# gnosisguild/stylus-zkvm-verifiers

Measured on AMD Instinct MI355X. Metric: Groth16 proofs verified/sec (BN254), higher is better.
Workload: dtype u32

## Files before the change

### stylus_zkvm_verifiers_amd/csrc/k_gt.hip

```cpp
#include "zkv_internal.h"

namespace zkv {

__global__ __launch_bounds__(64) void k_gt_bases(const VkRaw* __restrict__ raw, const VkTables* __restrict__ t, uint32_t* __restrict__ tab, uint32_t* __restrict__ mconst,
                                                 uint32_t* __restrict__ scratch, uint32_t nw0, uint32_t nw1) {
    if (threadIdx.x != 0) return;
    const uint32_t b = blockIdx.x;
    uint32_t* sc = scratch + (size_t)b * 12 * 96;
    MRef fm = m_ref(sc, 1), tm = m_ref(sc + 96, 1), E = m_ref(sc + 2 * 96, 1), Y1 = m_ref(sc + 3 * 96, 1), Y3 = m_ref(sc + 4 * 96, 1), Y4 = m_ref(sc + 5 * 96, 1),
         W = m_ref(sc + 6 * 96, 1), acc = m_ref(sc + 9 * 96, 1);
    Fp2 gx, gy;
    gx.c0 = fp_from_raw(raw->gamma[0]); gx.c1 = fp_from_raw(raw->gamma[1]);
    gy.c0 = fp_from_raw(raw->gamma[2]); gy.c1 = fp_from_raw(raw->gamma[3]);
    G1Norm n;
    n.lxs = n.lys = n.cxs = n.cys = fp_zero();
    if (b == 2) {
        MRef out = m_ref(mconst, 1), ab = m_ref(const_cast<uint32_t*>(t->f_alpha_beta), 1);
        if (t->base_inf) { f12m_copy(out, ab); return; }
        const Fp iy = fp_inv(t->base.y);
        n.axs = fp_mul(t->base.x, iy); n.ays = iy;
        miller_loop_m((const VkTables*)nullptr, 0, n, gx, gy, fm, tm);
        f12m_mul(out, fm, ab);
        return;
    }
    const uint32_t nw = b ? nw1 : nw0, row0 = b ? nw0 : 0u;
    const uint32_t ici = raw->var_ic[b];
    const Fp px = fp_from_raw(raw->ic[ici][0]), py = fp_from_raw(raw->ic[ici][1]);
    const Fp iy = fp_inv(py);
    n.axs = fp_mul(px, iy); n.ays = iy;
    miller_loop_m((const VkTables*)nullptr, 0, n, gx, gy, fm, tm);
    (void)final_exp_is_one_m(fm, E, Y1, Y3, Y4, W, acc);
#pragma unroll 1
    for (uint32_t j = 0; j < nw; j++) {
        f12m_copy(m_ref(tab + gt_row_word(row0 + j), 1), acc);
#pragma unroll 1
        for (uint32_t k = 0; k < GT_WINDOW_BITS; k++) f12m_cyclo_sqr(acc);
    }
}

__global__ __launch_bounds__(64) void k_gt_level(uint32_t* __restrict__ tab, uint32_t rows, uint32_t level) {
    const uint32_t cnt = level == GT_WINDOW_BITS - 1 ? 1u : 1u << level;
    const uint32_t tt = blockIdx.x * 64 + threadIdx.x, row = blockIdx.y;
    if (tt >= cnt || row >= rows) return;
    const uint32_t d = (1u << level) + tt;
    uint32_t* base = tab + gt_row_word(row);
    MRef dst = m_ref(base + (size_t)(d - 1) * GT_ENTRY_WORDS, 1), src = m_ref(base + (size_t)((d >> 1) - 1) * GT_ENTRY_WORDS, 1), one = m_ref(base, 1);
    f12m_copy(dst, src);
    f12m_cyclo_sqr(dst);
    if (d & 1u) f12m_mul(dst, dst, one);
}

void launch_gt_bases(const VkRaw* d_raw, const VkTables* d_tab, uint32_t* tab, uint32_t* mconst, uint32_t* scratch, uint32_t nw0, uint32_t nw1, hipStream_t s) {
    hipLaunchKernelGGL(k_gt_bases, dim3(3), dim3(64), 0, s, d_raw, d_tab, tab, mconst, scratch, nw0, nw1);
}
void launch_gt_level(uint32_t* tab, uint32_t rows, uint32_t level, hipStream_t s) {
    if (!rows || level < 1 || level >= GT_WINDOW_BITS) return;
    const uint32_t cnt = level == GT_WINDOW_BITS - 1 ? 1u : 1u << level;
    hipLaunchKernelGGL(k_gt_level, dim3((cnt + 63) / 64, rows), dim3(64), 0, s, tab, rows, level);
}

}
```

### stylus_zkvm_verifiers_amd/csrc/zkv_capi.hip

```cpp
#include <hip/hip_runtime.h>
#include <condition_variable>
#include <functional>
#include <memory>
#include <mutex>
#include <new>
#include <math.h>
#include <stdio.h>
#include <stdlib.h>
#include <string.h>
#include <system_error>
#include <thread>
#include <utility>
#include <vector>

#include "../../include/zkv.h"
#include "../../include/zkv_groth16_set.h"
#include "../../include/zkv_sp1_gateway.h"
#include "../../include/zkv_sp1_gateway_wire.h"
#include "../../include/zkv_sp1_gateway_keys.h"
#include "../../include/zkv_plonk_keys.h"
#include "../../include/zkv_plonk_set.h"
#include "../../include/zkv_plonk_set_agg.h"
#include "../../include/zkv_diag_primitive.h"
#include "../../include/zkv_diag_prep.h"
// ... 429 lines not shown
        hipMalloc(&c->ws.f, sizeof(uint32_t) * WS_F_WORDS * cap) != hipSuccess ||
        hipMalloc(&c->ws.fe, sizeof(uint32_t) * WS_FE_WORDS * cap) != hipSuccess ||
        hipMalloc(&c->ws.flags, sizeof(uint32_t) * cap) != hipSuccess || hipMalloc(&c->ws.g2bad, sizeof(uint32_t) * cap) != hipSuccess ||
        hipMalloc(&c->d_a, 32 * cap) != hipSuccess || hipMalloc(&c->d_b, 32 * cap) != hipSuccess ||
        hipMalloc(&c->d_status, cap) != hipSuccess || hipMalloc(&c->d_recv, 4 * cap) != hipSuccess ||
        hipMalloc(&c->d_off, sizeof(uint64_t) * (cap + 1)) != hipSuccess ||
        hipMalloc(&c->d_pvoff, sizeof(uint64_t) * (cap + 1)) != hipSuccess ||
        hipMalloc(&c->d_inst_idx, sizeof(uint32_t) * cap) != hipSuccess ||
        hipMalloc(&c->d_len, sizeof(uint32_t) * cap) != hipSuccess || hipMalloc(&c->d_pvlen, sizeof(uint32_t) * cap) != hipSuccess ||
        hipMalloc(&c->d_kind, cap) != hipSuccess || hipMalloc(&c->d_cdoff[0], sizeof(uint64_t) * (cap + 1)) != hipSuccess ||
        hipMalloc(&c->d_cdoff[1], sizeof(uint64_t) * (cap + 1)) != hipSuccess ||
        ((is_plonk(c) || c->vm == ZKV_VM_PLONK_SET) && hipMalloc(&c->d_plonk_tab, sizeof(uint32_t) * PLONK_TAB_WORDS * cap) != hipSuccess)) {
        (void)hipGetLastError();
        return ZKV_ERR_OOM;
    }
    c->ws.cap = cap;
    return agg_reserve(c);
}
static int gt_window_bits() {
    const char* e = getenv("ZKV_GT_WINDOW_BITS");
    if (!e || !strcmp(e, "20")) return (int)GT_WINDOW_BITS;
    return !strcmp(e, "0") ? 0 : -1;
}
static size_t gt_max_bytes() {
    const char* e = getenv("ZKV_GT_MAX_BYTES");
    return e ? (size_t)strtoull(e, nullptr, 10) : ~(size_t)0;
}
static int gt_maybe_build(zkv_ctx* c, size_t n) {
    if (c->gt_tried || (c->vm != ZKV_VM_SP1 && c->vm != ZKV_VM_RISC0) || c->vk_invalid || !c->d_tab) return ZKV_OK;
    const size_t per = n < chunk_capacity() ? n : chunk_capacity();
    if (!(c->lanes == 2 || (c->lanes == 0 && per > wide_below()))) return ZKV_OK;
    const int bits = gt_window_bits();
    if (bits < 0) return ZKV_ERR_INVALID_ARG;
    c->gt_tried = true;
    if (bits == 0) return ZKV_OK;
    VkRaw raw;
    if (c->vm == ZKV_VM_RISC0) host::fill_vk_risc0(raw, c->control_root_0, c->control_root_1, c->control_id);
    else host::fill_vk_sp1(raw);
    if (raw.n_var != GT_MAX_SIG || !raw.var_windows[0] || !raw.var_windows[1]) return ZKV_OK;
    const uint32_t nw0 = gt_windows(8 * raw.var_windows[0]), nw1 = gt_windows(8 * raw.var_windows[1]), rows = nw0 + nw1;
    if (nw0 > GT_MAX_WINDOWS || nw1 > GT_MAX_WINDOWS) return ZKV_OK;
    const size_t bytes = (size_t)rows * GT_ROW_BYTES;
    if (bytes > gt_max_bytes()) return ZKV_OK;
    VkRaw* d_raw = nullptr; uint32_t* d_scr = nullptr;
    hipEvent_t e0 = nullptr, e1 = nullptr;
    bool ok = hipMalloc(&c->d_gt, bytes) == hipSuccess && hipMalloc(&c->d_gt_const, sizeof(uint32_t) * GT_ENTRY_WORDS) == hipSuccess &&
              hipMalloc(&d_raw, sizeof(VkRaw)) == hipSuccess && hipMalloc(&d_scr, sizeof(uint32_t) * GT_SETUP_SCRATCH_WORDS) == hipSuccess &&
              hipEventCreate(&e0) == hipSuccess && hipEventCreate(&e1) == hipSuccess;
    if (ok) {
        ok = hipMemcpyAsync(d_raw, &raw, sizeof raw, hipMemcpyHostToDevice, c->stream) == hipSuccess;
        (void)hipEventRecord(e0, c->stream);
        launch_gt_bases(d_raw, c->d_tab, c->d_gt, c->d_gt_const, d_scr, nw0, nw1, c->stream);
        for (uint32_t level = 1; level < GT_WINDOW_BITS; level++) launch_gt_level(c->d_gt, rows, level, c->stream);
        (void)hipEventRecord(e1, c->stream);
        ok = ok && hipGetLastError() == hipSuccess && hipStreamSynchronize(c->stream) == hipSuccess;
        if (ok) (void)hipEventElapsedTime(&c->gt_build_ms, e0, e1);
    }
    (void)hipGetLastError();
    if (e0) (void)hipEventDestroy(e0);
    if (e1) (void)hipEventDestroy(e1);
    if (d_raw) (void)hipFree(d_raw);
    if (d_scr) (void)hipFree(d_scr);
    if (!ok) {
        if (c->d_gt) (void)hipFree(c->d_gt);
        if (c->d_gt_const) (void)hipFree(c->d_gt_const);
        c->d_gt = c->d_gt_const = nullptr;
        return ZKV_OK;
    }
    c->gt = GtTab{c->d_gt, c->d_gt_const, {nw0, nw1}};
    c->gt_bytes = bytes;
    return ZKV_OK;
}
static int ctx_ready(zkv_ctx* c, size_t n, bool verify = true) {
    int rc = ctx_device_init(c);
    if (rc == ZKV_OK) rc = ctx_reserve(c, n ? n : 1);
    if (rc == ZKV_OK && verify) rc = gt_maybe_build(c, n ? n : 1);
    return rc;
}
static int grow(uint8_t** p, size_t* cap, size_t need) {
    if (need <= *cap) return ZKV_OK;
    if (*p) (void)hipFree(*p);
    *p = nullptr; *cap = 0;
    size_t want = need + need / 4 + 4096;
    if (hipMalloc(p, want) != hipSuccess) { (void)hipGetLastError(); return ZKV_ERR_OOM; }
    *cap = want;
    return ZKV_OK;
}

static int order_after_previous(zkv_ctx* c, hipStream_t s) {
    if (c->has_done) HIP_TRY(hipStreamWaitEvent(s, c->ev_done, 0));
    c->agg_look = true;
    return ZKV_OK;
}
static int mark_done(zkv_ctx* c, hipStream_t s) {
    HIP_TRY(hipEventRecord(c->ev_done, s));
    c->has_done = true;
    return ZKV_OK;
}

static size_t agg_min() {
    const char* e = getenv("ZKV_AGG_MIN");
    size_t v = e ? (size_t)strtoull(e, nullptr, 10) : (size_t)131072;
    return v < 64 ? 64 : v;
}
static uint32_t agg_group(uint32_t sub) {
    const char* e = getenv("ZKV_AGG_GROUP");
// ... 2547 lines not shown
    return rc;
}

static_assert(ZKV_DIAG_PREP_SIGNALS == MAX_VAR, "zkv_diag_prep.h documents MAX_VAR signal rows");
ZKV_EXPORT int zkv_diag_prep_signals(zkv_ctx* c, size_t n, uint32_t* signals, uint32_t* flags) {
    if (!c || !signals || !flags || n == 0) return ZKV_ERR_INVALID_ARG;
    if (is_sharded(c) || (c->vm != ZKV_VM_RISC0 && c->vm != ZKV_VM_SP1) || c->agg_on) return ZKV_ERR_INVALID_ARG;
    int nd = 0;
    if (hipGetDeviceCount(&nd) != hipSuccess || nd <= 0) { (void)hipGetLastError(); return ZKV_ERR_NO_DEVICE; }
    if (c->device < 0 || c->device >= nd || !device_is_gfx950(c->device)) return ZKV_ERR_NO_DEVICE;
    std::lock_guard<std::mutex> lk(c->mu);
    if (!c->dev_ready || !c->ws.prep || n > c->last_chunk_n || n > c->ws.cap) return ZKV_ERR_INVALID_ARG;
    HIP_TRY(hipSetDevice(c->device));
    HIP_TRY(hipDeviceSynchronize());
    const size_t rows = (size_t)8 * MAX_VAR;
    std::vector<uint32_t> t(rows * n);
    HIP_TRY(hipMemcpy2D(t.data(), 4 * n, c->ws.prep + (size_t)64 * c->ws.cap, 4 * c->ws.cap, 4 * n, rows, hipMemcpyDeviceToHost));
    HIP_TRY(hipMemcpy(flags, c->ws.flags, 4 * n, hipMemcpyDeviceToHost));
    for (size_t j = 0; j < n; j++)
        for (size_t r = 0; r < rows; r++) signals[j * rows + r] = t[r * n + j];
    return ZKV_OK;
}

ZKV_EXPORT int zkv_ctx_vm(const zkv_ctx* c) { return c ? c->vm : ZKV_ERR_INVALID_ARG; }
ZKV_EXPORT int zkv_ctx_set_lanes_per_proof(zkv_ctx* c, int lanes) {
    if (!c || (lanes != 0 && lanes != 2 && lanes != 16 && lanes != 64 && lanes != 128)) return ZKV_ERR_INVALID_ARG;
    if (is_sharded(c)) { for (auto* k : c->shards) { const int rc = zkv_ctx_set_lanes_per_proof(k, lanes); if (rc != ZKV_OK) return rc; } return ZKV_OK; }
    if (c->vm == ZKV_VM_MIXED) {
        for (auto* k : c->kid) { const int rc = zkv_ctx_set_lanes_per_proof(k, lanes); if (rc != ZKV_OK) return rc; }
    }
    for (auto* k : c->gw_route) { if (!k) continue; const int rc = zkv_ctx_set_lanes_per_proof(k, lanes); if (rc != ZKV_OK) return rc; }
    if (c->gw_group) { const int rc = zkv_ctx_set_lanes_per_proof(c->gw_group, lanes); if (rc != ZKV_OK) return rc; }
    std::lock_guard<std::mutex> lk(c->mu);
    c->lanes = lanes;
    return ZKV_OK;
}
ZKV_EXPORT int zkv_diag_gt_info(zkv_ctx* c, uint64_t* out6) {
    if (!c || !out6) return ZKV_ERR_INVALID_ARG;
    std::lock_guard<std::mutex> lk(c->mu);
    out6[0] = c->gt.tab ? 1 : 0; out6[1] = c->gt.nw[0]; out6[2] = c->gt.nw[1]; out6[3] = c->gt_bytes;
    out6[4] = (uint64_t)(c->gt_build_ms * 1000.0f); out6[5] = c->gt_tried ? 1 : 0;
    return ZKV_OK;
}
ZKV_EXPORT int zkv_diag_gt_read(zkv_ctx* c, int signal, uint32_t window, uint32_t d, uint32_t* out96) {
    if (!c || !out96) return ZKV_ERR_INVALID_ARG;
    std::lock_guard<std::mutex> lk(c->mu);
    if (!c->gt.tab) return ZKV_ERR_INVALID_ARG;
    if (hipSetDevice(c->device) != hipSuccess) return ZKV_ERR_HIP;
    const uint32_t* src = c->gt.mconst;
    if (signal >= 0) {
        if (signal >= (int)GT_MAX_SIG || window >= c->gt.nw[signal] || d < 1 || d > GT_ROW_ENTRIES) return ZKV_ERR_INVALID_ARG;
        src = c->gt.tab + gt_row_word((signal ? c->gt.nw[0] : 0u) + window) + gt_entry_offset(d) / 4;
    }
    HIP_TRY(hipMemcpy(out96, src, sizeof(uint32_t) * GT_ENTRY_WORDS, hipMemcpyDeviceToHost));
    return ZKV_OK;
}
ZKV_EXPORT int zkv_diag_gt_product(zkv_ctx* c, size_t n, const uint32_t* scalars, uint32_t* out) {
    if (!c || !n || !scalars || !out) return ZKV_ERR_INVALID_ARG;
    std::lock_guard<std::mutex> lk(c->mu);
    if (!c->gt.tab || n > c->ws.cap) return ZKV_ERR_INVALID_ARG;
    for (size_t i = 0; i < n; i++) for (uint32_t sig = 0; sig < GT_MAX_SIG; sig++) {
        const uint32_t top = GT_WINDOW_BITS * c->gt.nw[sig] - 1u;
        for (uint32_t b = top; b < 256; b++) if ((scalars[(i * GT_MAX_SIG + sig) * 8 + (b >> 5)] >> (b & 31u)) & 1u) return ZKV_ERR_INVALID_ARG;
    }
    if (hipSetDevice(c->device) != hipSuccess) return ZKV_ERR_HIP;
    int rc = order_after_previous(c, c->stream);
    if (rc != ZKV_OK) return rc;
    constexpr size_t SW = 8 * GT_MAX_SIG;
    std::vector<uint32_t> rows(SW * n), res((size_t)GT_ENTRY_WORDS * n);
    for (size_t i = 0; i < n; i++) for (size_t k = 0; k < SW; k++) rows[k * n + i] = scalars[i * SW + k];
    uint8_t* d_st = nullptr;
    HIP_TRY(hipMalloc(&d_st, n));
    const size_t cap = c->ws.cap;
    bool ok = hipMemcpy2DAsync(c->ws.prep + 64 * cap, cap * 4, rows.data(), n * 4, n * 4, SW, hipMemcpyHostToDevice, c->stream) == hipSuccess;
    if (ok) {
        launch_gt_diag_seed(n, c->ws, c->stream);
        launch_finalexp2(n, c->ws, d_st, c->stream, c->gt);
        ok = hipGetLastError() == hipSuccess &&
             hipMemcpy2DAsync(res.data(), n * 4, c->ws.fe + (size_t)(96 * 6) * cap, cap * 4, n * 4, GT_ENTRY_WORDS, hipMemcpyDeviceToHost, c->stream) == hipSuccess &&
             hipStreamSynchronize(c->stream) == hipSuccess;
    }
    (void)hipFree(d_st);
    if (!ok) { (void)hipGetLastError(); return ZKV_ERR_HIP; }
    for (size_t i = 0; i < n; i++) for (size_t k = 0; k < GT_ENTRY_WORDS; k++) out[i * GT_ENTRY_WORDS + k] = res[k * n + i];
    return ZKV_OK;
}
ZKV_EXPORT int zkv_ctx_set_aggregate_check(zkv_ctx* c, int enable, const uint8_t* seed32) {
    if (!c || (enable != 0 && enable != 1 && enable != 16 && enable != 32 && enable != 64 && enable != 128 && enable != 256)) return ZKV_ERR_INVALID_ARG;
    uint8_t seed[32];
    if (enable) {
        if (seed32) memcpy(seed, seed32, 32);
        else if (getrandom(seed, 32, 0) != 32) return ZKV_ERR_INVALID_ARG;
    }
    if (is_sharded(c)) {
        for (size_t k = 0; k < c->shards.size(); k++) {
            uint8_t sk[32];
            if (enable && seed32) { uint8_t buf[36]; memcpy(buf, seed, 32); buf[32] = (uint8_t)(k >> 24); buf[33] = (uint8_t)(k >> 16); buf[34] = (uint8_t)(k >> 8); buf[35] = (uint8_t)k; host::sha256_host(buf, 36, sk); }
            const int rc = zkv_ctx_set_aggregate_check(c->shards[k], enable, enable && seed32 ? sk : nullptr);
            { volatile uint8_t* w = sk; for (int i = 0; i < 32; i++) w[i] = 0; }
            if (rc != ZKV_OK) return rc;
        }
        return ZKV_OK;
    }
    if (c->vm == ZKV_VM_MIXED || c->vm == ZKV_VM_SP1_GATEWAY) {
        const size_t nk = c->vm == ZKV_VM_MIXED ? 2 : c->gw_route.size();
        for (size_t k = 0; k < nk; k++) {
            if (c->vm == ZKV_VM_SP1_GATEWAY && !c->gw_route[k]) continue;
            uint8_t sk[32];
            if (enable && seed32) { uint8_t buf[33]; memcpy(buf, seed, 32); buf[32] = (uint8_t)k; host::sha256_host(buf, 33, sk); }
            const int rc = zkv_ctx_set_aggregate_check(c->vm == ZKV_VM_MIXED ? c->kid[k] : c->gw_route[k], enable, enable && seed32 ? sk : nullptr);
            { volatile uint8_t* w = sk; for (int i = 0; i < 32; i++) w[i] = 0; }
            if (rc != ZKV_OK) return rc;
        }
        return ZKV_OK;
    }
    if (c->vm != ZKV_VM_RISC0 && c->vm != ZKV_VM_RISC0_SET && c->vm != ZKV_VM_SP1 && c->vm != ZKV_VM_GROTH16 && c->vm != ZKV_VM_SP1_PLONK &&
        c->vm != ZKV_VM_GROTH16_SET && c->vm != ZKV_VM_PLONK && c->vm != ZKV_VM_PLONK_SET)
        return enable ? ZKV_ERR_INVALID_ARG : ZKV_OK;
    {
        std::lock_guard<std::mutex> lk(c->mu);
        c->agg_on = enable != 0;
        if (enable) {
            c->agg_auto = enable == 1; c->agg_sub = enable == 1 ? 32u : (uint32_t)enable;
            c->agg_resnap = c->dev_ready;
            if (!c->dev_ready) c->agg_seen[0] = c->agg_seen[1] = 0;
            c->agg_pause = c->agg_pause_len = 0;
            c->agg_os_seed = seed32 == nullptr; c->agg_key_age = 0;
            for (int i = 0; i < 8; i++) c->agg_seed.w[i] = be32_of(seed + 4 * i);
        }
    }
    volatile uint8_t* wipe = seed;
    for (int i = 0; i < 32; i++) wipe[i] = 0;
    return ZKV_OK;
}
ZKV_EXPORT int zkv_ctx_aggregate_counters(zkv_ctx* c, uint64_t out[2]) {
// ... 145 lines not shown
```

### stylus_zkvm_verifiers_amd/csrc/zkv_internal.h

```cpp
#pragma once
#include <hip/hip_runtime.h>
#include "zkv_verify.h"

namespace zkv {

constexpr int WS_PREP_WORDS = 64 + 8 * MAX_VAR;
constexpr int WS_NORM_WORDS = 48;
constexpr int WS_F_WORDS = 96;
constexpr int WS_FE_WORDS = 7 * 96;
struct Workspace {
    uint32_t* prep; uint32_t* norm; uint32_t* f; uint32_t* fe; uint32_t* flags;
    uint32_t* g2bad;
    size_t cap;
};

constexpr int ZKV_BLOCK = 64;

__device__ __forceinline__ Fp ws_ld(const uint32_t* base, size_t cap, int word0, size_t i) {
    Fp r;
#pragma unroll
    for (int k = 0; k < 8; k++) r.v[k] = base[(size_t)(word0 + k) * cap + i];
    return r;
}
__device__ __forceinline__ void ws_st(uint32_t* base, size_t cap, int word0, size_t i, const Fp& a) {
// ... 20 lines not shown
    const uint32_t* pv_len;
    const uint32_t* inst; const InstTab* inst_tab; uint32_t n_inst;
    uint32_t* plonk_tab;
    uint32_t not_initialized;
    uint8_t* status; uint8_t* recv;
};

struct WireArgs {
    size_t n;
    const uint8_t* cd;
    const uint64_t* off;
    uint64_t cd_bytes;
    uint32_t sel_a_be, sel_b_be;
    uint8_t* seals;
    uint32_t* seal_len;
    uint8_t* in_a; uint8_t* in_b;
    uint8_t* kind;
    uint8_t* pv; uint64_t* pv_off; uint32_t* pv_len;
};
void launch_wire_risc0(const WireArgs& a, hipStream_t s);
void launch_wire_sp1(const WireArgs& a, hipStream_t s);
struct GwWireArgs {
    size_t n;
    const uint8_t* cd; const uint64_t* off; uint64_t cd_bytes;
    uint32_t sel_u_be, sel_b_be;
    uint8_t* arena;
    uint64_t cd_delta, arena_delta;
    uint8_t* vkeys;
    uint64_t* pv_at; uint32_t* pv_len; uint64_t* proof_at; uint32_t* proof_len; uint8_t* bad;
};
void launch_wire_gateway(const GwWireArgs& a, hipStream_t s);

void launch_setup(const VkRaw* d_raw, VkTables* d_tab, hipStream_t s);
void launch_prep_risc0(const PrepArgs& a, const Risc0Consts& k, const Workspace& ws, hipStream_t s);
void launch_prep_sp1(const PrepArgs& a, const Workspace& ws, hipStream_t s);
void launch_prep_groth16(const PrepArgs& a, const Workspace& ws, hipStream_t s);
void launch_setup_msm16(const VkTables* d_tab, const Msm16& m, G1A* tab, uint32_t rows, hipStream_t s);
void launch_msm(size_t n, const VkTables* d_tab, const Msm16& m16, const InstTab* inst_tab, const Workspace& ws, hipStream_t s, bool skip_vk_x = false);
void launch_msm_w(size_t n, const VkTables* d_tab, const InstTab* inst_tab, const Workspace& ws, hipStream_t s);
void launch_setup_long(const uint32_t* d_ic, uint32_t n_sig, VkTables* d_tab, G1A* tab, uint32_t* win, hipStream_t s);
void launch_prep_groth16_long(const PrepArgs& a, const Workspace& ws, uint32_t* sig, size_t stride, hipStream_t s);
void launch_msm_long(size_t n, uint32_t lanes, const VkTables* d_tab, const LongKey& lk, const Workspace& ws, hipStream_t s);
void launch_vk_x_long(size_t n, uint32_t lanes, const VkTables* d_tab, const LongKey& lk, const uint8_t* sig, uint8_t* out, hipStream_t s);
void launch_status_to_bool(size_t n, uint8_t* status, hipStream_t s);
void launch_setup_instances(const VkRaw* d_raw, const InstConsts& k, const InstRaw* d_in, InstTab* d_out, uint32_t n_inst, hipStream_t s);
void launch_vk_x(size_t n, const VkTables* d_tab, const Msm16& m16, const InstTab* inst_tab, const uint32_t* inst, const uint8_t* sig, uint8_t* out, hipStream_t s);
void launch_g2chk2(size_t n, const Workspace& ws, uint8_t* status, hipStream_t s);
constexpr GtTab GT_NONE = {nullptr, nullptr, {0, 0}};
void launch_miller2(size_t n, const VkTables* d_tab, const Workspace& ws, uint8_t* status, hipStream_t s, const uint32_t* mconst = nullptr);
void launch_finalexp2(size_t n, const Workspace& ws, uint8_t* status, hipStream_t s, const GtTab& gt = GT_NONE);
constexpr size_t GT_SETUP_SCRATCH_WORDS = 3 * 12 * 96;
void launch_gt_bases(const VkRaw* d_raw, const VkTables* d_tab, uint32_t* tab, uint32_t* mconst, uint32_t* scratch, uint32_t nw0, uint32_t nw1, hipStream_t s);
void launch_gt_level(uint32_t* tab, uint32_t rows, uint32_t level, hipStream_t s);
void launch_gt_diag_seed(size_t n, const Workspace& ws, hipStream_t s);
void launch_miller_w(size_t n, const VkTables* d_tab, const Workspace& ws, hipStream_t s);
void launch_finalexp_w(size_t n, const Workspace& ws, uint8_t* status, hipStream_t s);
void launch_miller_w64(size_t n, const VkTables* d_tab, const Workspace& ws, hipStream_t s);
void launch_finalexp_w64(size_t n, const Workspace& ws, uint8_t* status, hipStream_t s);
void launch_miller_w64d(size_t n, const VkTables* d_tab, const Workspace& ws, uint8_t* status, hipStream_t s);

struct MixedArgs {
    size_t n;
    const uint8_t* vm;
    const uint8_t* method;
    const uint8_t* seals; const uint64_t* seal_off; uint32_t seal_stride;
    const uint8_t* in_a;
    const uint8_t* in_b; const uint64_t* b_off; uint32_t b_stride, pv_len;
    const uint32_t* cnt; const uint32_t* totals;
    uint32_t* pos; uint32_t* idx;
    uint8_t* c_seals; uint32_t* c_len; uint8_t* c_a; uint8_t* c_b; uint64_t* c_pvoff; uint32_t* c_pvlen;
    uint8_t* c_kind;
    uint8_t* status; uint8_t* recv;
};
void launch_mixed_partition(const MixedArgs& a, uint32_t* cnt, uint32_t* totals, hipStream_t s);
void launch_mixed_return(size_t m, const uint32_t* idx, const uint8_t* c_status, const uint8_t* c_recv, uint8_t* status, uint8_t* recv, hipStream_t s);

constexpr int GW_MAX_ROUTES = 8, GW_COL_NOT_FOUND = 8, GW_COL_SHORT = 9, GW_COL_BAD = 10, GW_COLS = 11;
constexpr uint32_t GW_NONE = 0xFFFFFFFFu;
struct GatewayArgs {
    size_t n;
    const uint8_t* proofs; const uint64_t* proof_off; uint64_t proof_bytes;
    const uint8_t* vkeys;
    const uint64_t* pv_off; uint64_t pv_stride;
    const uint64_t* rec_proof_at; const uint32_t* rec_proof_len; const uint64_t* rec_pv_at; const uint32_t* rec_pv_len; const uint8_t* rec_bad;
    uint32_t n_routes;
    uint32_t sel[GW_MAX_ROUTES];
    uint32_t rec[GW_MAX_ROUTES];
    uint32_t start[GW_MAX_ROUTES]; uint64_t base[GW_MAX_ROUTES];
    uint32_t* cnt; uint32_t* totals;
    uint32_t* pos; uint32_t* idx;
    uint8_t* c_proofs; uint32_t* c_len; uint8_t* c_a; uint64_t* c_pvoff; uint32_t* c_pvlen;
    uint8_t* status; uint8_t* recv;
};
void launch_gateway_count(const GatewayArgs& a, hipStream_t s);
void launch_gateway_place(const GatewayArgs& a, hipStream_t s);

struct GsetKey { const VkTables* tab; uint32_t sig0, n_sig, negate, pad; };
constexpr uint32_t GSET_NONE = 0xFFFFFFFFu;
struct GsetPart {
    size_t n; uint32_t n_keys, blocks, per_block;
    const uint32_t* key;
    uint32_t* cnt;
    uint32_t* totals;
    uint32_t* off;
    uint32_t* idx; uint32_t* skey;
    uint32_t* pos;
// ... 98 lines not shown
```

### stylus_zkvm_verifiers_amd/csrc/zkv_tower_mem.h

```cpp
#pragma once
#include "zkv_curve.h"

namespace zkv {

struct MRef {
    uint32_t* p; uint32_t stride; uint32_t f2w;
    ZKV_HD uint32_t ld(int k) const { return p[(size_t)k * stride]; }
    ZKV_HD void st(int k, uint32_t v) const { p[(size_t)k * stride] = v; }
    ZKV_HD int fw() const { return (int)f2w; }
};
ZKV_HD MRef m_ref(uint32_t* p, uint32_t stride, uint32_t f2w = 16) { MRef r; r.p = p; r.stride = stride; r.f2w = f2w; return r; }
ZKV_HD MRef m_off(MRef m, int words) { MRef r = m; r.p = m.p + (size_t)words * m.stride; return r; }

struct SoaRW {
    uint32_t* p; size_t stride; uint32_t off;
    ZKV_HD uint32_t ld(int k) const { return *(const uint32_t*)((const char*)(p + (size_t)k * stride) + off); }
    ZKV_HD void st(int k, uint32_t v) const { *(uint32_t*)((char*)(p + (size_t)k * stride) + off) = v; }
    ZKV_HD int fw() const { return 16; }
};
template <class R> ZKV_HD R m_fresh(R r) { return r; }
ZKV_HD SoaRW m_fresh(SoaRW r) {
#if defined(__HIP_DEVICE_COMPILE__)
    asm volatile("" : "+v"(r.off));
#endif
// ... 198 lines not shown
        { const LTerm t[3] = {{raw.v0.l, 1}, {(const uint32_t*)raw.wa, 9}, {(const uint32_t*)pw, k1}}; xc0 = l9_lincomb(t, 48); }
        const L9 pv2 = l9_partner(raw.v2);
        { const LTerm t[3] = {{(const uint32_t*)raw.wb, 1}, {raw.v2.l, 9}, {pv2.l, k1}}; xc1 = l9_lincomb(t, 8); }
        { const LTerm t[1] = {{(const uint32_t*)raw.wc, 1}}; xc2 = l9_lincomb(t, 8); }
    }
    uint32_t xy0[9], xy1[9], xy2[9];
    {
        L9 g0, g1, g2;
        const RB S = m_fresh(S0);
        l9_f6_mul_raw([&](int i) { return l9_ld(acc, 3 + i); }, [&](int i) {
            Fp2 b = m_ld_f2(S, 3 + i);
            if (conj_b) b = f2_neg(b);
            return l9_from_fp(b.h);
        }, raw);
        L9 yc0, yc1, yc2;
        l9_partner_i32(raw.wa, pw);
        { const LTerm t[3] = {{raw.v0.l, 1}, {(const uint32_t*)raw.wa, 9}, {(const uint32_t*)pw, k1}}; yc0 = l9_lincomb(t, 48); }
        const L9 pv2 = l9_partner(raw.v2);
        { const LTerm t[3] = {{(const uint32_t*)raw.wb, 1}, {raw.v2.l, 9}, {pv2.l, k1}}; yc1 = l9_lincomb(t, 8); }
        { const LTerm t[1] = {{(const uint32_t*)raw.wc, 1}}; yc2 = l9_lincomb(t, 8); }
        const L9 pyc2 = l9_partner(yc2);
        { const LTerm t[3] = {{xc0.l, 1}, {yc2.l, 9}, {pyc2.l, k1}}; g0 = l9_lincomb(t, 4); }
        { const LTerm t[2] = {{xc1.l, 1}, {yc0.l, 1}}; g1 = l9_lincomb(t, 1); }
        { const LTerm t[2] = {{xc2.l, 1}, {yc1.l, 1}}; g2 = l9_lincomb(t, 1); }
#pragma unroll
        for (int i = 0; i < 9; i++) { xy0[i] = xc0.l[i] + yc0.l[i]; xy1[i] = xc1.l[i] + yc1.l[i]; xy2[i] = xc2.l[i] + yc2.l[i]; }
#pragma unroll
        for (int i = 0; i < 3; i++) {
            const L9 g = l9_ld(acc, i), h = l9_ld(acc, 3 + i);
            L9 sum;
#pragma unroll
            for (int k = 0; k < 9; k++) sum.l[k] = g.l[k] + h.l[k];
            l9_carry(sum.l);
            l9_st(acc, 3 + i, sum);
        }
        l9_st(acc, 0, g0); l9_st(acc, 1, g1); l9_st(acc, 2, g2);
    }
    L9 h0, h1, h2;
    {
        const RB S = m_fresh(S0);
        l9_f6_mul_raw([&](int i) { return l9_ld(acc, 3 + i); }, [&](int i) {
            Fp2 b = m_ld_f2(S, 3 + i);
            if (conj_b) b = f2_neg(b);
            return l9_from_fp(f2_add(m_ld_f2(S, i), b).h);
        }, raw);
        l9_partner_i32(raw.wa, pw);
        { const LTerm t[4] = {{raw.v0.l, 1}, {(const uint32_t*)raw.wa, 9}, {(const uint32_t*)pw, k1}, {xy0, -1}}; h0 = l9_lincomb(t, 52); }
        const L9 pv2 = l9_partner(raw.v2);
        { const LTerm t[4] = {{(const uint32_t*)raw.wb, 1}, {raw.v2.l, 9}, {pv2.l, k1}, {xy1, -1}}; h1 = l9_lincomb(t, 12); }
        { const LTerm t[2] = {{(const uint32_t*)raw.wc, 1}, {xy2, -1}}; h2 = l9_lincomb(t, 12); }
    }
    l9_st(acc, 3, h0); l9_st(acc, 4, h1); l9_st(acc, 5, h2);
}
#endif

template <class RD, class RA, class RB> ZKV_HD void f12m_mul_body(RD d, RA a, RB b, bool conj_b) {
    Fp6 ag = m_ld_f6(a, 0), bg = m_ld_f6(b, 0);
    Fp6 t0 = f6_mul(ag, bg);
    Fp6 ah = m_ld_f6(a, 3), bh = m_ld_f6(b, 3);
    if (conj_b) bh = f6_neg(bh);
    Fp6 t1 = f6_mul(ah, bh);
    Fp6 m = f6_mul(f6_add(ag, ah), f6_add(bg, bh));
    d = m_fresh(d);
    m_st_f6(d, 3, f6_sub(f6_sub(m, t0), t1));
    m_st_f6(d, 0, f6_add(t0, f6_mul_v(t1)));
}
template <class RD, class RA, class RB> ZKV_HD_NI void f12m_mul(RD d, RA a, RB b) { f12m_mul_body(d, a, b, false); }
template <class RD, class RA, class RB> ZKV_HD_NI void f12m_mul_conj(RD d, RA a, RB b) { f12m_mul_body(d, a, b, true); }
#if defined(ZKV_PAIRED)
template <class RF> ZKV_HD void f12m_mul_by_034_body(RF f, const Fp2& c0, const Fp2& c3, const Fp2& c4) {
    uint32_t c0U[9], c0V[9], c4U[9], c4V[9], tU[9], tV[9], xo[9], xp[9];
    f2_limbs_y(c0.h, c0U, c0V); f2_limbs_y(c4.h, c4U, c4V);
    Fp2 t0c0, t0c1, t0c2, t1c0, t1c1, t1c2;
    {
        const Fp2 h0 = m_ld_f2(f, 3), h1 = m_ld_f2(f, 4), h2 = m_ld_f2(f, 5);
        Fp2 p4, p5, p6, p7, p8;
        f2_limbs_y(c3.h, tU, tV);
        f2_limbs_x(h0.h, xo, xp); p4.h = f2_mul_limbs(xo, xp, tU, tV);
        f2_limbs_x(h2.h, xo, xp); p8.h = f2_mul_limbs(xo, xp, tU, tV); p7.h = f2_mul_limbs(xo, xp, c4U, c4V);
        f2_limbs_x(h1.h, xo, xp); p5.h = f2_mul_limbs(xo, xp, c4U, c4V);
        f2_limbs_y(f2_add_nr(c3, c4).h, tU, tV);
        f2_limbs_x(f2_add_nr(h0, h1).h, xo, xp); p6.h = f2_mul_limbs(xo, xp, tU, tV);
        t1c0 = f2_add(p4, f2_mul_xi(p7)); t1c1 = f2_sub(f2_sub(p6, p4), p5); t1c2 = f2_add(p5, p8);
    }
    Fp2 s0, s1, s2;
    {
        const Fp2 g0 = m_ld_f2(f, 0), g1 = m_ld_f2(f, 1), g2 = m_ld_f2(f, 2);
        f2_limbs_x(g0.h, xo, xp); t0c0.h = f2_mul_limbs(xo, xp, c0U, c0V);
        f2_limbs_x(g1.h, xo, xp); t0c1.h = f2_mul_limbs(xo, xp, c0U, c0V);
        f2_limbs_x(g2.h, xo, xp); t0c2.h = f2_mul_limbs(xo, xp, c0U, c0V);
        s0 = f2_add(g0, m_ld_f2(f, 3)); s1 = f2_add(g1, m_ld_f2(f, 4)); s2 = f2_add(g2, m_ld_f2(f, 5));
    }
    m_st_f2(f, 0, f2_add(t0c0, f2_mul_xi(t1c2))); m_st_f2(f, 1, f2_add(t0c1, t1c0)); m_st_f2(f, 2, f2_add(t0c2, t1c1));
    const Fp2 b0 = f2_add(c0, c3);
    Fp2 w0, w1, n, q;
    f2_limbs_y(b0.h, tU, tV);
    f2_limbs_x(s0.h, xo, xp); w0.h = f2_mul_limbs(xo, xp, tU, tV);
    f2_limbs_x(s2.h, xo, xp); q.h = f2_mul_limbs(xo, xp, tU, tV);
    Fp2 q2; q2.h = f2_mul_limbs(xo, xp, c4U, c4V);
    f2_limbs_x(s1.h, xo, xp); w1.h = f2_mul_limbs(xo, xp, c4U, c4V);
    f2_limbs_y(f2_add_nr(b0, c4).h, tU, tV);
    f2_limbs_x(f2_add_nr(s0, s1).h, xo, xp); n.h = f2_mul_limbs(xo, xp, tU, tV);
    m_st_f2(f, 3, f2_sub(f2_sub(f2_add(w0, f2_mul_xi(q2)), t0c0), t1c0));
    m_st_f2(f, 4, f2_sub(f2_sub(f2_sub(f2_sub(n, w0), w1), t0c1), t1c1));
    m_st_f2(f, 5, f2_sub(f2_sub(f2_add(w1, q), t0c2), t1c2));
}
// ... 87 lines not shown
```

### stylus_zkvm_verifiers_amd/csrc/zkv_verify.h

```cpp
#pragma once
#include "zkv_tower_mem.h"
#include "zkv_sha256.h"
#include "zkv_gt.h"

namespace zkv {

enum : uint8_t {
    ST_OK = 0, ST_VERIFICATION_FAILED = 1, ST_INVALID_INITIALIZATION = 2, ST_ALREADY_INITIALIZED = 3,
    ST_INVALID_PROOF_DATA = 4, ST_SELECTOR_MISMATCH = 5,
    ST_BAD_CALLDATA = 6
};
enum : uint32_t { FL_ALIVE = 1u, FL_A_INF = 2u, FL_B_INF = 4u, FL_C_INF = 8u, FL_L_INF = 16u };

constexpr int N_LINES = 88;
constexpr int MSM_MAX_WINDOWS = 32;
constexpr int MSM_DIGITS = 256;
constexpr int MAX_IC = 6;
constexpr int MAX_VAR = 5;

struct VkRaw {
    uint32_t alpha[2][8];
    uint32_t beta[4][8], gamma[4][8], delta[4][8];
    uint32_t ic[MAX_IC][2][8];
    uint32_t n_ic;
// ... 386 lines not shown
    f12m_mul(X17, acc, x);
    f12m_copy(acc, X17); f12m_cyclo_sqr(acc);
    f12m_mul(X35, acc, x);
    { const int t = u_digit(ZKV_U_DIG_LEN - 1); f12m_copy(acc, t == 1 ? x : t == 17 ? X17 : X35); }
#pragma unroll 1
    for (int i = ZKV_U_DIG_LEN - 2; i >= 0; i--) {
        f12m_cyclo_sqr(acc);
        const int d = u_digit(i);
        if (d == 0) continue;
        const int m = d < 0 ? -d : d;
        const MRef S = m == 1 ? x : m == 17 ? X17 : X35;
        if (d > 0) f12m_mul(acc, acc, S);
        else f12m_mul_conj(acc, acc, S);
    }
}
template <class RA> ZKV_HD bool final_exp_is_one_m(MRef F, MRef E, MRef Y1, MRef Y3, MRef Y4, MRef W, RA acc) {
    f12m_copy(acc, F); f12m_conj(acc);
    f12m_inv(F, F);
    f12m_mul(acc, acc, F);
    f12m_frob(F, acc, 2);
    f12m_mul(E, F, acc);
    exp_u_m(acc, E, W); f12m_conj(acc);
    f12m_cyclo_sqr(acc); f12m_copy(Y1, acc);
    f12m_cyclo_sqr(acc);
    f12m_mul(acc, acc, Y1); f12m_copy(Y3, acc);
    exp_u_m(acc, Y3, W); f12m_conj(acc); f12m_copy(Y4, acc);
    f12m_cyclo_sqr(acc); f12m_copy(F, acc);
    exp_u_m(acc, F, W);
    f12m_conj(Y3);
    f12m_mul(acc, acc, Y4);
    f12m_mul(acc, acc, Y3); f12m_copy(Y3, acc);
    f12m_mul(F, acc, Y1);
    f12m_mul(acc, acc, Y4);
    f12m_mul(acc, acc, E);
    f12m_frob(Y1, F, 1);
    f12m_mul(acc, Y1, acc);
    f12m_frob(Y3, Y3, 2);
    f12m_mul(acc, Y3, acc);
    f12m_conj(E);
    f12m_mul(E, E, F);
    f12m_frob(E, E, 3);
    f12m_mul(acc, E, acc);
    return f12m_is_one(acc);
}

#if defined(ZKV_PAIRED)
ZKV_HD SoaRW fe_slot(int s, uint32_t* fbase, uint32_t* ebase, size_t cap, uint32_t off) {
    SoaRW r; r.p = s == 1 ? fbase : ebase + (size_t)(96 * (s - 2)) * cap; r.stride = cap; r.off = off;
    return r;
}
struct GtRef { bool on; ptrdiff_t rel; const uint32_t* sc; uint32_t nw0, nw1; };
constexpr uint32_t FE_PROG_TAIL_CHECK[ZKV_FE_PROG_LEN] = ZKV_FE_PROG;
static_assert(FE_PROG_TAIL_CHECK[ZKV_FE_PROG_LEN - 2] == (0u | 8u << 8 | 0u << 16) && (FE_PROG_TAIL_CHECK[ZKV_FE_PROG_LEN - 1] & 0xffffu) == (7u | 8u << 8),
              "final_exp_prog_p: the table walk goes in front of the program's last two entries, COPY TMP <- ACC; ISONE TMP, with TMP = slot 8");
ZKV_HD bool zkv_wave_any(bool v) {
#if defined(__HIP_DEVICE_COMPILE__)
    return __builtin_amdgcn_ballot_w64(v) != 0;
#else
    return v;
#endif
}
ZKV_HD bool final_exp_prog_p(uint32_t* fbase, uint32_t* ebase, size_t cap, uint32_t off, L9Ref acc, const GtRef gt = GtRef{false, 0, nullptr, 0, 0}) {
    const uint32_t PROG[ZKV_FE_PROG_LEN] = ZKV_FE_PROG;
    const uint32_t GT_PROG[4] = {8u, 1u, 3u | 8u << 24, 1u};
    bool one = false;
    const uint32_t slot = zkv_wave_slot_parity();
    const int n_extra = gt.on ? 4 * (int)(gt.nw0 + gt.nw1) : 0, cut = ZKV_FE_PROG_LEN - 2;
#pragma unroll 1
    for (int pc = 0; pc < ZKV_FE_PROG_LEN + n_extra; pc++) {
        const int q = pc - cut;
        const bool extra = q >= 0 && q < n_extra;
        const uint32_t row = extra ? (uint32_t)q >> 2 : 0u;
        const uint32_t e = extra ? GT_PROG[q & 3] : PROG[q < 0 ? pc : pc - n_extra];
        const int op = (int)(e & 255u), d = (int)((e >> 8) & 255u), a = (int)((e >> 16) & 255u), b = (int)(e >> 24);
        if ((pc & 3) == 0) zkv_fair_share(slot);
#if defined(__HIP_DEVICE_COMPILE__)
        asm volatile("" : "+v"(off));
#endif
        int32_t dg = 0;
        if (extra) {
            const uint32_t sig = row >= gt.nw0 ? 1u : 0u, j = sig ? row - gt.nw0 : row, k = gt_digit_word(j);
            const uint32_t i4 = off - 32u * zkv_parity() * (uint32_t)cap;
            const uint32_t lo = *(const uint32_t*)((const char*)(gt.sc + (size_t)(8u * sig + k) * cap) + i4);
            const uint32_t hi = k + 1 < 8 ? *(const uint32_t*)((const char*)(gt.sc + (size_t)(8u * sig + k + 1) * cap) + i4) : 0u;
            dg = gt_digit_of(lo, hi, j);
            if (!zkv_wave_any(dg != 0)) continue;
        }
        if (op == 6) { ZKV_MARK("begin cyclo"); f12l9_cyclo_sqr(acc); ZKV_MARK("end cyclo"); }
        else if ((op == 3 || op == 4) && d == 0) { ZKV_MARK("begin accmul");  f12l9_mul(acc, fe_slot(b, fbase, ebase, cap, off), op == 4); ZKV_MARK("end accmul"); }
        else if (op == 8) {
            const SoaRW D = fe_slot(8, fbase, ebase, cap, off);
            if (dg == 0) f12m_set_one(D);
            else {
                SoaRW T;
                T.p = ebase + gt.rel + (ptrdiff_t)gt_row_word(row); T.stride = 1;
                T.off = gt_entry_offset((uint32_t)(dg < 0 ? -dg : dg)) + 32u * zkv_parity();
                f12m_copy(D, T);
            }
        }
        else if (op == 0 && d == 0) f12m_copy(acc, fe_slot(a, fbase, ebase, cap, off));
        else if (op == 0 && a == 0) f12m_copy(fe_slot(d, fbase, ebase, cap, off), acc);
        else if (op == 1 && d == 0) { if (!extra || dg < 0) f12m_conj(acc); }
        else {
            const SoaRW D = fe_slot(d, fbase, ebase, cap, off), A = fe_slot(a, fbase, ebase, cap, off);
            if (op == 3 || op == 4) { ZKV_MARK("begin genmul"); f12m_mul_body(D, A, fe_slot(b, fbase, ebase, cap, off), op == 4); ZKV_MARK("end genmul"); }
            else if (op == 0) f12m_copy(D, A);
            else if (op == 1) f12m_conj(D);
            else if (op == 2) { ZKV_MARK("begin geninv"); f12m_inv_body(D, A); ZKV_MARK("end geninv"); }
            else if (op == 5) { ZKV_MARK("begin genfrob"); f12m_frob_body(D, A, b); ZKV_MARK("end genfrob"); }
            else one = f12m_is_one(D);
        }
    }
    return one;
}
#endif

#if !defined(ZKV_PAIRED)
ZKV_HD bool raw_g1_is_inf(const uint32_t p[2][8]) { return raw_is_zero(p[0]) && raw_is_zero(p[1]); }
ZKV_HD bool raw_g1_valid(const uint32_t p[2][8]) {
    if (!raw_lt_p(p[0]) || !raw_lt_p(p[1])) return false;
    if (raw_g1_is_inf(p)) return true;
    return g1_on_curve(fp_from_raw(p[0]), fp_from_raw(p[1]));
}
ZKV_HD bool raw_g2_is_inf(const uint32_t q[4][8]) { return raw_is_zero(q[0]) && raw_is_zero(q[1]) && raw_is_zero(q[2]) && raw_is_zero(q[3]); }
ZKV_HD bool raw_g2_valid(const uint32_t q[4][8]) {
    for (int k = 0; k < 4; k++) if (!raw_lt_p(q[k])) return false;
    if (raw_g2_is_inf(q)) return true;
    Fp2 x, y; x.c0 = fp_from_raw(q[0]); x.c1 = fp_from_raw(q[1]); y.c0 = fp_from_raw(q[2]); y.c1 = fp_from_raw(q[3]);
    return g2_on_twist(x, y) && g2_in_subgroup(x, y);
}
ZKV_HD void setup_validate(const VkRaw& vk, VkTables& t) {
    bool ok = raw_g1_valid(vk.alpha) && raw_g2_valid(vk.beta) && raw_g2_valid(vk.gamma) && raw_g2_valid(vk.delta);
    for (uint32_t i = 0; i < vk.n_ic; i++) ok = ok && raw_g1_valid(vk.ic[i]);
    t.vk_valid = ok ? 1u : 0u;
    t.skip_fixed[0] = raw_g2_is_inf(vk.gamma) ? 1u : 0u;
    t.skip_fixed[1] = raw_g2_is_inf(vk.delta) ? 1u : 0u;
}
ZKV_HD LineAffC line_to_table(const LineAff& l) {
    LineAffC r; r.nl.c0 = l.nl.c0; r.nl.c1 = l.nl.c1; r.c.c0 = l.c.c0; r.c.c1 = l.c.c1; return r;
}
ZKV_HD void setup_lines(const uint32_t q[4][8], LineAffC* out) {
    if (raw_g2_is_inf(q)) return;
    G2A Q, T;
    Q.x.c0 = fp_from_raw(q[0]); Q.x.c1 = fp_from_raw(q[1]); Q.y.c0 = fp_from_raw(q[2]); Q.y.c1 = fp_from_raw(q[3]);
    T = Q;
    Fp2 nqy = f2_neg(Q.y);
    int li = 0;
#pragma unroll 1
    for (int i = ZKV_ATE_NAF_LEN - 2; i >= 0; i--) {
        out[li++] = line_to_table(aff_dbl(T));
        int d = ate_naf(i);
        if (d != 0) out[li++] = line_to_table(aff_add(T, Q.x, d > 0 ? Q.y : nqy));
    }
    Fp2 q1x, q1y, q2x, q2y;
    g2_frob_affine(q1x, q1y, Q.x, Q.y);
// ... 161 lines not shown
```

Before: 6.472 million.

## Store GT window table in torus-compressed form and use sparse accumulator multiply

After the GT window table is built, a new pass compresses each Fp12 entry to a 6-word torus representation (g+1)/h. The final-exponentiation table walk then loads only half an entry per window and multiplies the accumulator by (w + a·x)-style sparse elements, with no per-window conj and full mul. It replaces the final is-one check with a comparison of the accumulator against the conjugate of the saved value, which avoids a full Fp12 multiply. The cost is a more involved multiply kernel, a new compression pass at setup, and reworked diagnostics that must expand or ratio results back into standard form.

After: 6.661 million, median of 6. 2.9% higher.

```diff
diff --git a/stylus_zkvm_verifiers_amd/csrc/k_gt.hip b/stylus_zkvm_verifiers_amd/csrc/k_gt.hip
--- a/stylus_zkvm_verifiers_amd/csrc/k_gt.hip
+++ b/stylus_zkvm_verifiers_amd/csrc/k_gt.hip
@@ -50,6 +50,36 @@
     if (d & 1u) f12m_mul(dst, dst, one);
 }
 
+__global__ __launch_bounds__(64) void k_gt_torus(uint32_t* __restrict__ tab, uint32_t rows) {
+    const uint32_t e = blockIdx.x * 64 + threadIdx.x, row = blockIdx.y;
+    if (e >= GT_ROW_ENTRIES || row >= rows) return;
+    MRef t = m_ref(tab + gt_row_word(row) + (size_t)e * GT_ENTRY_WORDS, 1);
+    Fp6 g = m_ld_f6(t, 0);
+    const Fp6 h = m_ld_f6(t, 3);
+    g.c0 = f2_add(g.c0, f2_one());
+    m_st_f6(t, 0, f6_mul(g, f6_inv(h)));
+}
+
+__global__ __launch_bounds__(64) void k_gt_diag_expand(const uint32_t* __restrict__ a48, uint32_t* __restrict__ out96) {
+    if (blockIdx.x != 0 || threadIdx.x != 0) return;
+    MRef s = m_ref(const_cast<uint32_t*>(a48), 1), o = m_ref(out96, 1);
+    const Fp6 a = m_ld_f6(s, 0), q = f6_mul(a, a);
+    Fp6 num = q, den = q;
+    num.c1 = f2_add(q.c1, f2_one()); den.c1 = f2_sub(q.c1, f2_one());
+    const Fp6 di = f6_inv(den);
+    m_st_f6(o, 0, f6_mul(num, di));
+    m_st_f6(o, 3, f6_mul(f6_add(a, a), di));
+}
+__global__ __launch_bounds__(64) void k_gt_diag_ratio(size_t n, const uint32_t* __restrict__ tmp, size_t cap, uint32_t* __restrict__ out, uint32_t* __restrict__ scr) {
+    const size_t i = (size_t)blockIdx.x * 64 + threadIdx.x;
+    if (i >= n) return;
+    MRef u = m_ref(const_cast<uint32_t*>(tmp) + i, (uint32_t)cap), o = m_ref(out + i, (uint32_t)n), c = m_ref(scr + i, (uint32_t)n);
+    f12m_copy(c, u);
+    f12m_conj(c);
+    f12m_inv(c, c);
+    f12m_mul(o, u, c);
+}
+
 void launch_gt_bases(const VkRaw* d_raw, const VkTables* d_tab, uint32_t* tab, uint32_t* mconst, uint32_t* scratch, uint32_t nw0, uint32_t nw1, hipStream_t s) {
     hipLaunchKernelGGL(k_gt_bases, dim3(3), dim3(64), 0, s, d_raw, d_tab, tab, mconst, scratch, nw0, nw1);
 }
@@ -58,5 +88,16 @@
     const uint32_t cnt = level == GT_WINDOW_BITS - 1 ? 1u : 1u << level;
     hipLaunchKernelGGL(k_gt_level, dim3((cnt + 63) / 64, rows), dim3(64), 0, s, tab, rows, level);
 }
+void launch_gt_torus(uint32_t* tab, uint32_t rows, hipStream_t s) {
+    if (!rows) return;
+    hipLaunchKernelGGL(k_gt_torus, dim3(GT_ROW_ENTRIES / 64, rows), dim3(64), 0, s, tab, rows);
+}
+void launch_gt_diag_expand(const uint32_t* a48, uint32_t* out96, hipStream_t s) {
+    hipLaunchKernelGGL(k_gt_diag_expand, dim3(1), dim3(64), 0, s, a48, out96);
+}
+void launch_gt_diag_ratio(size_t n, const uint32_t* tmp, size_t cap, uint32_t* out, uint32_t* scr, hipStream_t s) {
+    if (!n) return;
+    hipLaunchKernelGGL(k_gt_diag_ratio, dim3((unsigned)((n + 63) / 64)), dim3(64), 0, s, n, tmp, cap, out, scr);
+}
 
 }
diff --git a/stylus_zkvm_verifiers_amd/csrc/zkv_capi.hip b/stylus_zkvm_verifiers_amd/csrc/zkv_capi.hip
--- a/stylus_zkvm_verifiers_amd/csrc/zkv_capi.hip
+++ b/stylus_zkvm_verifiers_amd/csrc/zkv_capi.hip
@@ -505,6 +505,7 @@
         (void)hipEventRecord(e0, c->stream);
         launch_gt_bases(d_raw, c->d_tab, c->d_gt, c->d_gt_const, d_scr, nw0, nw1, c->stream);
         for (uint32_t level = 1; level < GT_WINDOW_BITS; level++) launch_gt_level(c->d_gt, rows, level, c->stream);
+        launch_gt_torus(c->d_gt, rows, c->stream);
         (void)hipEventRecord(e1, c->stream);
         ok = ok && hipGetLastError() == hipSuccess && hipStreamSynchronize(c->stream) == hipSuccess;
         if (ok) (void)hipEventElapsedTime(&c->gt_build_ms, e0, e1);
@@ -3158,7 +3159,14 @@
         if (signal >= (int)GT_MAX_SIG || window >= c->gt.nw[signal] || d < 1 || d > GT_ROW_ENTRIES) return ZKV_ERR_INVALID_ARG;
         src = c->gt.tab + gt_row_word((signal ? c->gt.nw[0] : 0u) + window) + gt_entry_offset(d) / 4;
     }
-    HIP_TRY(hipMemcpy(out96, src, sizeof(uint32_t) * GT_ENTRY_WORDS, hipMemcpyDeviceToHost));
+    if (signal < 0) { HIP_TRY(hipMemcpy(out96, src, sizeof(uint32_t) * GT_ENTRY_WORDS, hipMemcpyDeviceToHost)); return ZKV_OK; }
+    uint32_t* d_out = nullptr;
+    HIP_TRY(hipMalloc(&d_out, sizeof(uint32_t) * GT_ENTRY_WORDS));
+    launch_gt_diag_expand(src, d_out, c->stream);
+    const bool ok = hipGetLastError() == hipSuccess && hipStreamSynchronize(c->stream) == hipSuccess &&
+                    hipMemcpy(out96, d_out, sizeof(uint32_t) * GT_ENTRY_WORDS, hipMemcpyDeviceToHost) == hipSuccess;
+    (void)hipFree(d_out);
+    if (!ok) { (void)hipGetLastError(); return ZKV_ERR_HIP; }
     return ZKV_OK;
 }
 ZKV_EXPORT int zkv_diag_gt_product(zkv_ctx* c, size_t n, const uint32_t* scalars, uint32_t* out) {
@@ -3176,17 +3184,20 @@
     std::vector<uint32_t> rows(SW * n), res((size_t)GT_ENTRY_WORDS * n);
     for (size_t i = 0; i < n; i++) for (size_t k = 0; k < SW; k++) rows[k * n + i] = scalars[i * SW + k];
     uint8_t* d_st = nullptr;
+    uint32_t* d_m = nullptr;
     HIP_TRY(hipMalloc(&d_st, n));
+    if (hipMalloc(&d_m, sizeof(uint32_t) * 2 * GT_ENTRY_WORDS * n) != hipSuccess) { (void)hipGetLastError(); (void)hipFree(d_st); return ZKV_ERR_HIP; }
     const size_t cap = c->ws.cap;
     bool ok = hipMemcpy2DAsync(c->ws.prep + 64 * cap, cap * 4, rows.data(), n * 4, n * 4, SW, hipMemcpyHostToDevice, c->stream) == hipSuccess;
     if (ok) {
         launch_gt_diag_seed(n, c->ws, c->stream);
         launch_finalexp2(n, c->ws, d_st, c->stream, c->gt);
+        launch_gt_diag_ratio(n, c->ws.fe + (size_t)(96 * 6) * cap, cap, d_m, d_m + (size_t)GT_ENTRY_WORDS * n, c->stream);
         ok = hipGetLastError() == hipSuccess &&
-             hipMemcpy2DAsync(res.data(), n * 4, c->ws.fe + (size_t)(96 * 6) * cap, cap * 4, n * 4, GT_ENTRY_WORDS, hipMemcpyDeviceToHost, c->stream) == hipSuccess &&
+             hipMemcpyAsync(res.data(), d_m, sizeof(uint32_t) * GT_ENTRY_WORDS * n, hipMemcpyDeviceToHost, c->stream) == hipSuccess &&
              hipStreamSynchronize(c->stream) == hipSuccess;
     }
-    (void)hipFree(d_st);
+    (void)hipFree(d_st); (void)hipFree(d_m);
     if (!ok) { (void)hipGetLastError(); return ZKV_ERR_HIP; }
     for (size_t i = 0; i < n; i++) for (size_t k = 0; k < GT_ENTRY_WORDS; k++) out[i * GT_ENTRY_WORDS + k] = res[k * n + i];
     return ZKV_OK;
diff --git a/stylus_zkvm_verifiers_amd/csrc/zkv_internal.h b/stylus_zkvm_verifiers_amd/csrc/zkv_internal.h
--- a/stylus_zkvm_verifiers_amd/csrc/zkv_internal.h
+++ b/stylus_zkvm_verifiers_amd/csrc/zkv_internal.h
@@ -96,6 +96,9 @@
 constexpr size_t GT_SETUP_SCRATCH_WORDS = 3 * 12 * 96;
 void launch_gt_bases(const VkRaw* d_raw, const VkTables* d_tab, uint32_t* tab, uint32_t* mconst, uint32_t* scratch, uint32_t nw0, uint32_t nw1, hipStream_t s);
 void launch_gt_level(uint32_t* tab, uint32_t rows, uint32_t level, hipStream_t s);
+void launch_gt_torus(uint32_t* tab, uint32_t rows, hipStream_t s);
+void launch_gt_diag_expand(const uint32_t* a48, uint32_t* out96, hipStream_t s);
+void launch_gt_diag_ratio(size_t n, const uint32_t* tmp, size_t cap, uint32_t* out, uint32_t* scr, hipStream_t s);
 void launch_gt_diag_seed(size_t n, const Workspace& ws, hipStream_t s);
 void launch_miller_w(size_t n, const VkTables* d_tab, const Workspace& ws, hipStream_t s);
 void launch_finalexp_w(size_t n, const Workspace& ws, uint8_t* status, hipStream_t s);
diff --git a/stylus_zkvm_verifiers_amd/csrc/zkv_tower_mem.h b/stylus_zkvm_verifiers_amd/csrc/zkv_tower_mem.h
--- a/stylus_zkvm_verifiers_amd/csrc/zkv_tower_mem.h
+++ b/stylus_zkvm_verifiers_amd/csrc/zkv_tower_mem.h
@@ -274,6 +274,58 @@
     }
     l9_st(acc, 3, h0); l9_st(acc, 4, h1); l9_st(acc, 5, h2);
 }
+ZKV_HD void l9_pin(L9& a) {
+#if defined(__HIP_DEVICE_COMPILE__)
+#pragma unroll
+    for (int i = 0; i < 9; i++) asm volatile("" : "+v"(a.l[i]));
+#else
+    (void)a;
+#endif
+}
+template <class RB> ZKV_HD void f12l9_mul_aw(L9Ref acc, RB S0, const bool neg, const bool keep) {
+    const int32_t k1 = zkv_parity() != 0 ? 1 : -1;
+    const int32_t sg = neg ? -1 : 1, sg9 = 9 * sg, sgk = k1 * sg;
+    L9F6Raw raw;
+    int32_t pw[9];
+    L9 n0, n1, n2;
+    {
+        const RB S = m_fresh(S0);
+        l9_f6_mul_raw([&](int i) { return l9_ld(acc, i); }, [&](int i) { return l9_from_fp(m_ld_f2(S, i).h); }, raw);
+        l9_partner_i32(raw.wa, pw);
+        const L9 d2 = l9_ld(acc, 5), pd2 = l9_partner(d2);
+        { const LTerm t[5] = {{raw.v0.l, sg}, {(const uint32_t*)raw.wa, sg9}, {(const uint32_t*)pw, sgk}, {d2.l, 9}, {pd2.l, k1}}; n0 = l9_lincomb(t, 48); }
+        const L9 pv2 = l9_partner(raw.v2), d0 = l9_ld(acc, 3);
+        { const LTerm t[4] = {{(const uint32_t*)raw.wb, sg}, {raw.v2.l, sg9}, {pv2.l, sgk}, {d0.l, 1}}; n1 = l9_lincomb(t, 28); }
+        const L9 d1 = l9_ld(acc, 4);
+        { const LTerm t[2] = {{(const uint32_t*)raw.wc, sg}, {d1.l, 1}}; n2 = l9_lincomb(t, 8); }
+    }
+    l9_pin(n0); l9_pin(n1); l9_pin(n2);
+    L9 h0, h1, h2;
+    {
+        const RB S = m_fresh(S0);
+        l9_f6_mul_raw([&](int i) { return l9_ld(acc, 3 + i); }, [&](int i) { return l9_from_fp(m_ld_f2(S, i).h); }, raw);
+        l9_partner_i32(raw.wa, pw);
+        const L9 g0 = l9_ld(acc, 0);
+        { const LTerm t[4] = {{raw.v0.l, sg}, {(const uint32_t*)raw.wa, sg9}, {(const uint32_t*)pw, sgk}, {g0.l, 1}}; h0 = l9_lincomb(t, 48); }
+        const L9 pv2 = l9_partner(raw.v2), g1 = l9_ld(acc, 1);
+        { const LTerm t[4] = {{(const uint32_t*)raw.wb, sg}, {raw.v2.l, sg9}, {pv2.l, sgk}, {g1.l, 1}}; h1 = l9_lincomb(t, 28); }
+        const L9 g2 = l9_ld(acc, 2);
+        { const LTerm t[2] = {{(const uint32_t*)raw.wc, sg}, {g2.l, 1}}; h2 = l9_lincomb(t, 8); }
+    }
+    if (keep) {
+        l9_st(acc, 0, n0); l9_st(acc, 1, n1); l9_st(acc, 2, n2);
+        l9_st(acc, 3, h0); l9_st(acc, 4, h1); l9_st(acc, 5, h2);
+    }
+}
+template <class RA, class RT> ZKV_HD bool f12m_eq_conj(RA a, RT t) {
+    bool ok = true;
+#pragma unroll 1
+    for (int k = 0; k < 6; k++) {
+        const Fp2 x = m_ld_f2(a, k), y = m_ld_f2(t, k);
+        ok = (k < 3 ? f2_eq(x, y) : f2_is_zero(f2_add(x, y))) && ok;
+    }
+    return ok;
+}
 #endif
 
 template <class RD, class RA, class RB> ZKV_HD void f12m_mul_body(RD d, RA a, RB b, bool conj_b) {
diff --git a/stylus_zkvm_verifiers_amd/csrc/zkv_verify.h b/stylus_zkvm_verifiers_amd/csrc/zkv_verify.h
--- a/stylus_zkvm_verifiers_amd/csrc/zkv_verify.h
+++ b/stylus_zkvm_verifiers_amd/csrc/zkv_verify.h
@@ -462,7 +462,7 @@
 struct GtRef { bool on; ptrdiff_t rel; const uint32_t* sc; uint32_t nw0, nw1; };
 constexpr uint32_t FE_PROG_TAIL_CHECK[ZKV_FE_PROG_LEN] = ZKV_FE_PROG;
 static_assert(FE_PROG_TAIL_CHECK[ZKV_FE_PROG_LEN - 2] == (0u | 8u << 8 | 0u << 16) && (FE_PROG_TAIL_CHECK[ZKV_FE_PROG_LEN - 1] & 0xffffu) == (7u | 8u << 8),
-              "final_exp_prog_p: the table walk goes in front of the program's last two entries, COPY TMP <- ACC; ISONE TMP, with TMP = slot 8");
+              "final_exp_prog_p: the table walk takes the place of the program's last two entries, COPY TMP <- ACC; ISONE TMP, with TMP = slot 8");
 ZKV_HD bool zkv_wave_any(bool v) {
 #if defined(__HIP_DEVICE_COMPILE__)
     return __builtin_amdgcn_ballot_w64(v) != 0;
@@ -472,23 +472,24 @@
 }
 ZKV_HD bool final_exp_prog_p(uint32_t* fbase, uint32_t* ebase, size_t cap, uint32_t off, L9Ref acc, const GtRef gt = GtRef{false, 0, nullptr, 0, 0}) {
     const uint32_t PROG[ZKV_FE_PROG_LEN] = ZKV_FE_PROG;
-    const uint32_t GT_PROG[4] = {8u, 1u, 3u | 8u << 24, 1u};
+    const uint32_t GT_PROG[7] = {0u | 5u << 8, 10u, 8u, 9u, 0u | 8u << 8, 3u | 5u << 24, 11u | 8u << 8};
     bool one = false;
     const uint32_t slot = zkv_wave_slot_parity();
-    const int n_extra = gt.on ? 4 * (int)(gt.nw0 + gt.nw1) : 0, cut = ZKV_FE_PROG_LEN - 2;
-#pragma unroll 1
-    for (int pc = 0; pc < ZKV_FE_PROG_LEN + n_extra; pc++) {
-        const int q = pc - cut;
-        const bool extra = q >= 0 && q < n_extra;
-        const uint32_t row = extra ? (uint32_t)q >> 2 : 0u;
-        const uint32_t e = extra ? GT_PROG[q & 3] : PROG[q < 0 ? pc : pc - n_extra];
+    const int cut = ZKV_FE_PROG_LEN - 2, n_win = gt.on ? 2 * (int)(gt.nw0 + gt.nw1) : 0;
+    const int n_prog = gt.on ? cut + 2 + n_win + 3 : ZKV_FE_PROG_LEN;
+#pragma unroll 1
+    for (int pc = 0; pc < n_prog; pc++) {
+        const int q = pc - cut - 2;
+        const bool extra = gt.on && pc >= cut, win = extra && q >= 0 && q < n_win;
+        const uint32_t row = win ? (uint32_t)q >> 1 : 0u;
+        const uint32_t e = !extra ? PROG[pc] : GT_PROG[q < 0 ? q + 2 : win ? 2 + (q & 1) : q - n_win + 4];
         const int op = (int)(e & 255u), d = (int)((e >> 8) & 255u), a = (int)((e >> 16) & 255u), b = (int)(e >> 24);
         if ((pc & 3) == 0) zkv_fair_share(slot);
 #if defined(__HIP_DEVICE_COMPILE__)
         asm volatile("" : "+v"(off));
 #endif
         int32_t dg = 0;
-        if (extra) {
+        if (win) {
             const uint32_t sig = row >= gt.nw0 ? 1u : 0u, j = sig ? row - gt.nw0 : row, k = gt_digit_word(j);
             const uint32_t i4 = off - 32u * zkv_parity() * (uint32_t)cap;
             const uint32_t lo = *(const uint32_t*)((const char*)(gt.sc + (size_t)(8u * sig + k) * cap) + i4);
@@ -498,19 +499,22 @@
         }
         if (op == 6) { ZKV_MARK("begin cyclo"); f12l9_cyclo_sqr(acc); ZKV_MARK("end cyclo"); }
         else if ((op == 3 || op == 4) && d == 0) { ZKV_MARK("begin accmul");  f12l9_mul(acc, fe_slot(b, fbase, ebase, cap, off), op == 4); ZKV_MARK("end accmul"); }
+        else if (op == 9) { ZKV_MARK("begin awmul"); f12l9_mul_aw(acc, fe_slot(8, fbase, ebase, cap, off), dg < 0, dg != 0); ZKV_MARK("end awmul"); }
         else if (op == 8) {
-            const SoaRW D = fe_slot(8, fbase, ebase, cap, off);
-            if (dg == 0) f12m_set_one(D);
-            else {
+            if (dg != 0) {
+                const SoaRW D = fe_slot(8, fbase, ebase, cap, off);
                 SoaRW T;
                 T.p = ebase + gt.rel + (ptrdiff_t)gt_row_word(row); T.stride = 1;
                 T.off = gt_entry_offset((uint32_t)(dg < 0 ? -dg : dg)) + 32u * zkv_parity();
-                f12m_copy(D, T);
+#pragma unroll 1
+                for (int k = 0; k < 3; k++) m_st_f2(D, k, m_ld_f2(T, k));
             }
         }
+        else if (op == 10) f12m_set_one(acc);
+        else if (op == 11) one = f12m_eq_conj(acc, fe_slot(d, fbase, ebase, cap, off));
         else if (op == 0 && d == 0) f12m_copy(acc, fe_slot(a, fbase, ebase, cap, off));
         else if (op == 0 && a == 0) f12m_copy(fe_slot(d, fbase, ebase, cap, off), acc);
-        else if (op == 1 && d == 0) { if (!extra || dg < 0) f12m_conj(acc); }
+        else if (op == 1 && d == 0) f12m_conj(acc);
         else {
             const SoaRW D = fe_slot(d, fbase, ebase, cap, off), A = fe_slot(a, fbase, ebase, cap, off);
             if (op == 3 || op == 4) { ZKV_MARK("begin genmul"); f12m_mul_body(D, A, fe_slot(b, fbase, ebase, cap, off), op == 4); ZKV_MARK("end genmul"); }
```
